# DavidHan008/SLAM-1

Measured on AMD Instinct MI355X. Metric: frames/sec tracking+local-BA @1280x720, higher is better.
Workload: dtype u8+f32+f64

## Files before the change

slam-1_amd/csrc/ba.hip:

```cpp
#include "common.hpp"

#include <cmath>

namespace {

typedef double d4 __attribute__((ext_vector_type(4)));

__device__ __forceinline__ void st_sc1(double* p, double v) {
  __hip_atomic_store(p, v, __ATOMIC_RELAXED, __HIP_MEMORY_SCOPE_AGENT);
}
__device__ __forceinline__ double ld_sc1(const double* p) {
  return __hip_atomic_load(const_cast<double*>(p), __ATOMIC_RELAXED, __HIP_MEMORY_SCOPE_AGENT);
}
__device__ __forceinline__ unsigned ticket_add(uint32_t* p) {
  return __hip_atomic_fetch_add(p, 1u, __ATOMIC_RELAXED, __HIP_MEMORY_SCOPE_AGENT);
}
__device__ __forceinline__ void ticket_reset(uint32_t* p) {
  __hip_atomic_store(p, 0u, __ATOMIC_RELAXED, __HIP_MEMORY_SCOPE_AGENT);
}

constexpr double kClamp = 5000.0;
constexpr double kDiagMin = 1e-6, kDiagMax = 1e32;
constexpr double kLamMin = 1e-16, kLamMax = 1e32;
constexpr int kBS = 256;
// ... 37 lines not shown
  const double omc = 1.0 - c;
  double R[3][3];
  R[0][0] = c + omc * v0 * v0; R[0][1] = -s * v2 + omc * v0 * v1; R[0][2] = s * v1 + omc * v0 * v2;
  R[1][0] = s * v2 + omc * v1 * v0; R[1][1] = c + omc * v1 * v1; R[1][2] = -s * v0 + omc * v1 * v2;
  R[2][0] = -s * v1 + omc * v2 * v0; R[2][1] = s * v0 + omc * v2 * v1; R[2][2] = c + omc * v2 * v2;
  const double th2 = w0 * w0 + w1 * w1 + w2 * w2;
  const double W[3][3] = {{0.0, -w2, w1}, {w2, 0.0, -w0}, {-w1, w0, 0.0}};
  const double w[3] = {w0, w1, w2};
  double A[3][3];
  for (int i = 0; i < 3; ++i)
    for (int k = 0; k < 3; ++k) {
      double acc = w[i] * w[k];
      for (int j = 0; j < 3; ++j) acc += R[j][i] * W[j][k];
      A[i][k] = acc - W[i][k];
    }
  o[0] = c; o[1] = s; o[2] = omc;
  o[3] = v0; o[4] = v1; o[5] = v2;
  for (int i = 0; i < 9; ++i) o[6 + i] = R[i / 3][i % 3];
  for (int i = 0; i < 9; ++i) o[15 + i] = A[i / 3][i % 3];
  o[24] = th2 < 1e-24 ? 0.0 : -1.0 / th2;
  o[25] = th2 < 1e-24 ? 1.0 : 0.0;
  for (int i = 0; i < 6; ++i) o[26 + i] = cam[3 + i];
}

template <bool JAC>
__device__ __forceinline__ void reproject_pre(const double* __restrict__ cr,
                                              const double* __restrict__ X,
                                              const double* __restrict__ q, double r[2],
                                              double J[2][12]) {
  const double c = cr[0], s = cr[1], omc = cr[2];
  const double v0 = cr[3], v1 = cr[4], v2 = cr[5];
  const double X0 = X[0], X1 = X[1], X2 = X[2];
  const double dot = X0 * v0 + X1 * v1 + X2 * v2;
  const double cx0 = v1 * X2 - v2 * X1;
  const double cx1 = v2 * X0 - v0 * X2;
  const double cx2 = v0 * X1 - v1 * X0;
  const double dk = dot * omc;
  const double RX0 = c * X0 + s * cx0 + dk * v0;
  const double RX1 = c * X1 + s * cx1 + dk * v1;
  const double RX2 = c * X2 + s * cx2 + dk * v2;
  const double P0 = RX0 + cr[26], P1 = RX1 + cr[27], P2 = RX2 + cr[28];
  const double p0 = -P0 / P2, p1 = -P1 / P2;
  const double f = cr[29], k1 = cr[30], k2 = cr[31];
  const double n = p0 * p0 + p1 * p1;
  const double rad = 1.0 + k1 * n + k2 * (n * n);
  const double sc = rad * f;
  r[0] = p0 * sc - q[0];
  r[1] = p1 * sc - q[1];
  if constexpr (JAC) {
    double R[3][3], A[3][3];
    for (int i = 0; i < 9; ++i) {
      R[i / 3][i % 3] = cr[6 + i];
      A[i / 3][i % 3] = cr[15 + i];
    }
    double dR[3][3];
    if (cr[25] != 0.0) {
      dR[0][0] = 0.0;  dR[0][1] = RX2;  dR[0][2] = -RX1;
      dR[1][0] = -RX2; dR[1][1] = 0.0;  dR[1][2] = RX0;
      dR[2][0] = RX1;  dR[2][1] = -RX0; dR[2][2] = 0.0;
    } else {
      const double Xs[3][3] = {{0.0, -X2, X1}, {X2, 0.0, -X0}, {-X1, X0, 0.0}};
      double B[3][3];
      for (int i = 0; i < 3; ++i)
        for (int k = 0; k < 3; ++k)
          B[i][k] = Xs[i][0] * A[0][k] + Xs[i][1] * A[1][k] + Xs[i][2] * A[2][k];
      const double inv = cr[24];
      for (int i = 0; i < 3; ++i)
        for (int k = 0; k < 3; ++k)
          dR[i][k] = (R[i][0] * B[0][k] + R[i][1] * B[1][k] + R[i][2] * B[2][k]) * inv;
    }
    const double iz = 1.0 / P2;
    const double dpP[2][3] = {{-iz, 0.0, P0 * iz * iz}, {0.0, -iz, P1 * iz * iz}};
    const double g2 = 2.0 * f * (k1 + 2.0 * k2 * n);
    const double Dp[2][2] = {{sc + g2 * p0 * p0, g2 * p0 * p1}, {g2 * p1 * p0, sc + g2 * p1 * p1}};
    double D[2][3];
    for (int a = 0; a < 2; ++a)
      for (int k = 0; k < 3; ++k) D[a][k] = Dp[a][0] * dpP[0][k] + Dp[a][1] * dpP[1][k];
    const double pp[2] = {p0, p1};
    for (int a = 0; a < 2; ++a) {
      for (int k = 0; k < 3; ++k) {
        J[a][k] = D[a][0] * dR[0][k] + D[a][1] * dR[1][k] + D[a][2] * dR[2][k];
        J[a][3 + k] = D[a][k];
        J[a][9 + k] = D[a][0] * R[0][k] + D[a][1] * R[1][k] + D[a][2] * R[2][k];
      }
      J[a][6] = pp[a] * rad;
      J[a][7] = pp[a] * (f * n);
      J[a][8] = pp[a] * (f * n * n);
    }
  }
}

template <bool JAC>
__device__ __forceinline__ void reproject(const double* __restrict__ cam,
                                          const double* __restrict__ X,
                                          const double* __restrict__ q, double r[2],
                                          double J[2][12]) {
  double cr[kCamRec];
  cam_prep(cam, cr);
  reproject_pre<JAC>(cr, X, q, r, J);
}

template <bool JAC>
__device__ __forceinline__ void clamp_rows(double r[2], double J[2][12]) {
#pragma unroll
  for (int comp = 0; comp < 2; ++comp) {
    const double rc = r[comp];
    if (fabs(rc) > kClamp) {
      const double arc = fabs(rc);
      const double half = comp == 0 ? 613.0 : 185.0;
      if constexpr (JAC) {
        const double a = (half * 2.0) / arc;
        double Jc[12];
        for (int k = 0; k < 12; ++k) Jc[k] = J[comp][k];
        for (int row = 0; row < 2; ++row) {
          const double ratio = r[row] / rc;
          for (int k = 0; k < 12; ++k) J[row][k] = a * (J[row][k] - ratio * Jc[k]);
        }
      }
      r[0] = r[0] / arc * half * 2.0;
      r[1] = r[1] / arc * half * 2.0;
    }
  }
}

__device__ __forceinline__ void hold_cols(double J[2][12], unsigned fx) {
#pragma unroll
  for (int i = 0; i < 9; ++i)
    if ((fx >> i) & 1u) J[0][i] = J[1][i] = 0.0;
}
template <int H>
__device__ __forceinline__ void hold_cols_half(double Jh[2][6], unsigned fx) {
#pragma unroll
  for (int i = 0; i < (H == 0 ? 6 : 3); ++i)
    if ((fx >> (6 * H + i)) & 1u) Jh[0][i] = Jh[1][i] = 0.0;
}

template <int H>
__device__ __forceinline__ void reproject_half(const double* __restrict__ cr,
                                               const double* __restrict__ X,
                                               const double* __restrict__ q, double r[2],
                                               double Jh[2][6]) {
  const double c = cr[0], s = cr[1], omc = cr[2];
  const double v0 = cr[3], v1 = cr[4], v2 = cr[5];
  const double X0 = X[0], X1 = X[1], X2 = X[2];
  const double dot = X0 * v0 + X1 * v1 + X2 * v2;
  const double cx0 = v1 * X2 - v2 * X1;
  const double cx1 = v2 * X0 - v0 * X2;
  const double cx2 = v0 * X1 - v1 * X0;
  const double dk = dot * omc;
  const double RX0 = c * X0 + s * cx0 + dk * v0;
  const double RX1 = c * X1 + s * cx1 + dk * v1;
  const double RX2 = c * X2 + s * cx2 + dk * v2;
  const double P0 = RX0 + cr[26], P1 = RX1 + cr[27], P2 = RX2 + cr[28];
  const double p0 = -P0 / P2, p1 = -P1 / P2;
  const double f = cr[29], k1 = cr[30], k2 = cr[31];
  const double n = p0 * p0 + p1 * p1;
  const double rad = 1.0 + k1 * n + k2 * (n * n);
  const double sc = rad * f;
  r[0] = p0 * sc - q[0];
  r[1] = p1 * sc - q[1];
  const double iz = 1.0 / P2;
  const double dpP[2][3] = {{-iz, 0.0, P0 * iz * iz}, {0.0, -iz, P1 * iz * iz}};
  const double g2 = 2.0 * f * (k1 + 2.0 * k2 * n);
  const double Dp[2][2] = {{sc + g2 * p0 * p0, g2 * p0 * p1}, {g2 * p1 * p0, sc + g2 * p1 * p1}};
  double D[2][3];
  for (int a = 0; a < 2; ++a)
    for (int k = 0; k < 3; ++k) D[a][k] = Dp[a][0] * dpP[0][k] + Dp[a][1] * dpP[1][k];
  if constexpr (H == 0) {
    double dR[3][3];
    if (cr[25] != 0.0) {
      dR[0][0] = 0.0;  dR[0][1] = RX2;  dR[0][2] = -RX1;
      dR[1][0] = -RX2; dR[1][1] = 0.0;  dR[1][2] = RX0;
      dR[2][0] = RX1;  dR[2][1] = -RX0; dR[2][2] = 0.0;
    } else {
      double R[3][3], A[3][3];
      for (int i = 0; i < 9; ++i) {
        R[i / 3][i % 3] = cr[6 + i];
        A[i / 3][i % 3] = cr[15 + i];
      }
      const double Xs[3][3] = {{0.0, -X2, X1}, {X2, 0.0, -X0}, {-X1, X0, 0.0}};
      double B[3][3];
      for (int i = 0; i < 3; ++i)
        for (int k = 0; k < 3; ++k)
          B[i][k] = Xs[i][0] * A[0][k] + Xs[i][1] * A[1][k] + Xs[i][2] * A[2][k];
      const double inv = cr[24];
      for (int i = 0; i < 3; ++i)
        for (int k = 0; k < 3; ++k)
          dR[i][k] = (R[i][0] * B[0][k] + R[i][1] * B[1][k] + R[i][2] * B[2][k]) * inv;
    }
    for (int a = 0; a < 2; ++a)
      for (int k = 0; k < 3; ++k) {
        Jh[a][k] = D[a][0] * dR[0][k] + D[a][1] * dR[1][k] + D[a][2] * dR[2][k];
        Jh[a][3 + k] = D[a][k];
      }
  } else {
    double R[3][3];
    for (int i = 0; i < 9; ++i) R[i / 3][i % 3] = cr[6 + i];
    const double pp[2] = {p0, p1};
    for (int a = 0; a < 2; ++a) {
      Jh[a][0] = pp[a] * rad;
      Jh[a][1] = pp[a] * (f * n);
      Jh[a][2] = pp[a] * (f * n * n);
      for (int k = 0; k < 3; ++k) Jh[a][3 + k] = D[a][0] * R[0][k] + D[a][1] * R[1][k] + D[a][2] * R[2][k];
    }
  }
#pragma unroll
  for (int comp = 0; comp < 2; ++comp) {
    const double rc = r[comp];
    if (fabs(rc) > kClamp) {
      const double arc = fabs(rc);
      const double half = comp == 0 ? 613.0 : 185.0;
      const double a = (half * 2.0) / arc;
      double Jc[6];
      for (int k = 0; k < 6; ++k) Jc[k] = Jh[comp][k];
      for (int row = 0; row < 2; ++row) {
        const double ratio = r[row] / rc;
        for (int k = 0; k < 6; ++k) Jh[row][k] = a * (Jh[row][k] - ratio * Jc[k]);
      }
      r[0] = r[0] / arc * half * 2.0;
      r[1] = r[1] / arc * half * 2.0;
    }
  }
}

__device__ __forceinline__ double block_sum(double v, double* lds) {
  for (int off = 32; off > 0; off >>= 1) v += __shfl_down(v, off, 64);
  const int lane = threadIdx.x & 63, wid = threadIdx.x >> 6;
  if (lane == 0) lds[wid] = v;
  __syncthreads();
  double s = 0.0;
  if (threadIdx.x == 0) {
    const int nw = (blockDim.x + 63) >> 6;
    for (int w = 0; w < nw; ++w) s += lds[w];
  }
  __syncthreads();
  return s;
}

__global__ __launch_bounds__(kBS) void k_residual(const double* __restrict__ cams,
                                                  const double* __restrict__ pts,
                                                  const int32_t* __restrict__ ci,
                                                  const int32_t* __restrict__ pi,
                                                  const double* __restrict__ qs, int n_obs,
                                                  double* __restrict__ resid,
                                                  double* __restrict__ jac) {
  const int o = blockIdx.x * kBS + threadIdx.x;
  if (o >= n_obs) return;
  double r[2], J[2][12];
  if (jac) {
    reproject<true>(cams + 9 * ci[o], pts + 3 * pi[o], qs + 2 * o, r, J);
    clamp_rows<true>(r, J);
    for (int a = 0; a < 2; ++a)
      for (int k = 0; k < 12; ++k) jac[(size_t)o * 24 + a * 12 + k] = J[a][k];
  } else {
    reproject<false>(cams + 9 * ci[o], pts + 3 * pi[o], qs + 2 * o, r, J);
    clamp_rows<false>(r, J);
  }
  resid[2 * o] = r[0];
  resid[2 * o + 1] = r[1];
}

__device__ __forceinline__ int cur_of(const double* state) {
  return state[SLAM_BA_ST_CUR] != 0.0 ? 1 : 0;
}

__device__ __forceinline__ double clampd(double d) { return fmin(fmax(d, kDiagMin), kDiagMax); }

constexpr int kDenseMaxN = 120;
__host__ __device__ __forceinline__ bool sys_packed(int n_cams) { return 9 * n_cams > kDenseMaxN; }
__host__ __device__ __forceinline__ long long sys_vec_off(int n_cams, int n_blocks) {
  return sys_packed(n_cams) ? 81ll * n_blocks : 81ll * n_cams * n_cams;
}


struct PtSchur {
  double V00 = 0, V01 = 0, V02 = 0, V11 = 0, V12 = 0, V22 = 0, g0 = 0, g1 = 0, g2 = 0;
  double d[3], iv[6], e[3];
  __device__ __forceinline__ void acc(double j0, double j1, double j2, double rr) {
    V00 += j0 * j0; V01 += j0 * j1; V02 += j0 * j2;
    V11 += j1 * j1; V12 += j1 * j2; V22 += j2 * j2;
    g0 -= j0 * rr; g1 -= j1 * rr; g2 -= j2 * rr;
  }
  __device__ __forceinline__ void solve(double lam);
};
__device__ __forceinline__ void PtSchur::solve(double lam) {
  d[0] = clampd(V00); d[1] = clampd(V11); d[2] = clampd(V22);
  const double a00 = V00 + lam * d[0], a11 = V11 + lam * d[1], a22 = V22 + lam * d[2];
  const double a01 = V01, a02 = V02, a12 = V12;
  const double c00 = a11 * a22 - a12 * a12;
  const double c01 = a02 * a12 - a01 * a22;
  const double c02 = a01 * a12 - a02 * a11;
  const double c11 = a00 * a22 - a02 * a02;
  const double c12 = a01 * a02 - a00 * a12;
  const double c22 = a00 * a11 - a01 * a01;
  const double det = a00 * c00 + a01 * c01 + a02 * c02;
  const double id = det != 0.0 ? 1.0 / det : 0.0;
  iv[0] = c00 * id; iv[1] = c01 * id; iv[2] = c02 * id;
  iv[3] = c11 * id; iv[4] = c12 * id; iv[5] = c22 * id;
  e[0] = iv[0] * g0 + iv[1] * g1 + iv[2] * g2;
  e[1] = iv[1] * g0 + iv[3] * g1 + iv[4] * g2;
  e[2] = iv[2] * g0 + iv[4] * g1 + iv[5] * g2;
}

constexpr int kCPart = 112;
constexpr int kGrp = 128;
constexpr int kLinWG = 256;
constexpr int kSlotLds = 128;
constexpr int kPairLds = 1024;

struct LinLds {
  double jc[kGrp][18];
  double w[kGrp][27];
  double ru[kGrp][4];
  double pt[kGrp][9];
  int lpt[kGrp];
  int cobs[kGrp];
  int cptr[kSlotLds];
  int bptr[kSlotLds];
  int pairs[kPairLds];
  unsigned fx[kGrp];
};

__device__ __forceinline__ void y_row(const double* W, const double* Vi, int i, double y[3]) {
  const double a = W[3 * i], b = W[3 * i + 1], c = W[3 * i + 2];
  y[0] = a * Vi[0] + b * Vi[1] + c * Vi[2];
  y[1] = a * Vi[1] + b * Vi[3] + c * Vi[4];
  y[2] = a * Vi[2] + b * Vi[4] + c * Vi[5];
}

__device__ __forceinline__ void lin_slots(const slam_ba_problem& p, LinLds& L, int cs0, int ncs,
                                          int bs0, int nbs, const int* cptr, int coff,
                                          const int* bptr, int boff, const int* pairs) {
  const int t = threadIdx.x;
  const int* cobs = L.cobs;
  for (int item = t; item < 9 * (ncs + nbs); item += kLinWG) {
    const int sl = item / 9, i = item - 9 * sl;
    double acc[9];
#pragma unroll
    for (int j = 0; j < 9; ++j) acc[j] = 0.0;
    if (sl < ncs) {
      const int s = cs0 + sl;
      double vr = 0.0, vu = 0.0, vd = 0.0, cost = 0.0;
      const int qb = cptr[sl] - coff, qe = cptr[sl + 1] - coff;
      int k = cobs[qb < qe ? qb : 0], lk = L.lpt[k];
      for (int q = qb; q < qe; ++q) {
        const int kn = cobs[q + 1 < qe ? q + 1 : q], lkn = L.lpt[kn];
        const double* jc = L.jc[k];
        const double* W = L.w[k];
        double y[3];
        y_row(W, L.pt[lk] + 3, i, y);
        const double a0 = jc[i], a1 = jc[9 + i];
#pragma unroll
        for (int j = 0; j < 9; ++j) {
          const double u = __builtin_fma(a0, jc[j], a1 * jc[9 + j]);
          const double v = __builtin_fma(y[0], W[3 * j], __builtin_fma(y[1], W[3 * j + 1], y[2] * W[3 * j + 2]));
          acc[j] += u - v;
        }
        const double r0 = L.ru[k][0], r1 = L.ru[k][1];
        vr = __builtin_fma(a0, r0, __builtin_fma(a1, r1, vr));
        vu = __builtin_fma(a0, L.ru[k][2], __builtin_fma(a1, L.ru[k][3], vu));
        vd = __builtin_fma(a0, a0, __builtin_fma(a1, a1, vd));
        cost = __builtin_fma(r0, r0, __builtin_fma(r1, r1, cost));
        k = kn;
        lk = lkn;
      }
      double* out = p.cpart + (size_t)p.cslot_row[s] * kCPart;
#pragma unroll
      for (int j = 0; j < 9; ++j) out[9 * i + j] = acc[j];
      out[81 + i] = vr;
      out[90 + i] = vu;
      out[99 + i] = vd;
      if (i == 0) out[108] = cost;
    } else {
      const int sb = sl - ncs, s = bs0 + sb;
      const int qb = bptr[sb] - boff, qe = bptr[sb + 1] - boff;
      int pr = pairs[qb < qe ? qb : 0], lk = L.lpt[pr & 0xffff];
      for (int q = qb; q < qe; ++q) {
        const int prn = pairs[q + 1 < qe ? q + 1 : q], lkn = L.lpt[prn & 0xffff];
        const int k1 = pr & 0xffff, k2 = pr >> 16;
        double y[3];
        y_row(L.w[k1], L.pt[lk] + 3, i, y);
        const double* W2 = L.w[k2];
#pragma unroll
        for (int j = 0; j < 9; ++j)
          acc[j] = __builtin_fma(y[0], W2[3 * j], __builtin_fma(y[1], W2[3 * j + 1], __builtin_fma(y[2], W2[3 * j + 2], acc[j])));
        pr = prn;
        lk = lkn;
      }
      double* out = p.bpart + (size_t)p.bslot_row[s] * 81;
#pragma unroll
      for (int j = 0; j < 9; ++j) out[9 * i + j] = acc[j];
    }
  }
}

#ifdef SLAM_LIN_PROFILE
#define LIN_T(i) const uint64_t lin_t##i = __builtin_amdgcn_s_memtime()
#else
#define LIN_T(i) (void)0
#endif
__global__ __launch_bounds__(kLinWG) void k_linearize(BaBatch bat) {
  BA_PROB_X(bat);
  const int g = bx;
  if (g >= p.n_grps) return;
  lm_wave_priority();
  __shared__ LinLds L;
  LIN_T(0);
  const int p0 = p.grp_ptr[g], p1 = p.grp_ptr[g + 1];
  const int o0 = p.pt_ptr[p0], o1 = p.pt_ptr[p1];
  const int t = threadIdx.x;
  const int o = o0 + t;
  const bool has = t < kGrp && o < o1;
  const int cur = cur_of(p.state);
  const int cs0 = p.grp_cslot[g], ncs = p.grp_cslot[g + 1] - cs0;
  const int bs0 = p.grp_bslot[g], nbs = p.grp_bslot[g + 1] - bs0;
  const int cb0 = p.cslot_obs_ptr[cs0], pb0 = p.bslot_pair_ptr[bs0];
  const int npairs = p.bslot_pair_ptr[bs0 + nbs] - pb0;
  const bool fit_c = ncs < kSlotLds, fit_b = nbs < kSlotLds, fit_p = npairs <= kPairLds;
  if (fit_c && t <= ncs) L.cptr[t] = p.cslot_obs_ptr[cs0 + t] - cb0;
  if (fit_b && t <= nbs) L.bptr[t] = p.bslot_pair_ptr[bs0 + t] - pb0;
  if (t < kGrp && t < o1 - o0) L.cobs[t] = p.cslot_obs[cb0 + t];
  if (fit_p)
    for (int q = t; q < npairs; q += kLinWG) L.pairs[q] = p.bslot_pairs[pb0 + q];
  double r[2], J[2][12];
  if (has) {
    const int pt = p.obs_pt[o];
    reproject_pre<true>(p.camrec[cur] + kCamRec * p.obs_cam[o], p.pts[cur] + 3 * pt,
                        p.obs_q + 2 * o, r, J);
    clamp_rows<true>(r, J);
#pragma unroll
    for (int a = 0; a < 2; ++a) {
#pragma unroll
      for (int i = 0; i < 9; ++i) L.jc[t][9 * a + i] = J[a][i];
#pragma unroll
      for (int c = 0; c < 3; ++c) L.w[t][3 * a + c] = J[a][9 + c];
      L.w[t][6 + a] = r[a];
      L.ru[t][a] = r[a];
    }
    L.lpt[t] = pt - p0;
  }
  __syncthreads();
  if (p.cam_fixed != nullptr) {
    for (int sl = t; sl < ncs; sl += kLinWG) {
      const unsigned fx = p.cam_fixed[p.cslot_cam[cs0 + sl]];
      const int qe = p.cslot_obs_ptr[cs0 + sl + 1] - cb0;
      for (int q = p.cslot_obs_ptr[cs0 + sl] - cb0; q < qe; ++q) L.fx[L.cobs[q]] = fx;
    }
    __syncthreads();
    if (has) {
      const unsigned fx = L.fx[t];
      if (fx) {
        hold_cols(J, fx);
#pragma unroll
        for (int i = 0; i < 9; ++i)
          if ((fx >> i) & 1u) L.jc[t][i] = L.jc[t][9 + i] = 0.0;
      }
    }
  }
  LIN_T(1);
  const double lam = p.state[SLAM_BA_ST_LAMBDA];
  if (t < p1 - p0) {
    const int pt = p0 + t;
    PtSchur ps;
    for (int k = p.pt_ptr[pt] - o0; k < p.pt_ptr[pt + 1] - o0; ++k) {
#pragma unroll
      for (int a = 0; a < 2; ++a) ps.acc(L.w[k][3 * a], L.w[k][3 * a + 1], L.w[k][3 * a + 2], L.w[k][6 + a]);
    }
    ps.solve(lam);
#pragma unroll
    for (int k = 0; k < 3; ++k) L.pt[t][k] = ps.e[k];
#pragma unroll
    for (int k = 0; k < 6; ++k) L.pt[t][3 + k] = ps.iv[k];
  }
  __syncthreads();
  if (has) {
    const double* e = L.pt[L.lpt[t]];
#pragma unroll
    for (int i = 0; i < 9; ++i)
#pragma unroll
      for (int c = 0; c < 3; ++c) L.w[t][3 * i + c] = J[0][i] * J[0][9 + c] + J[1][i] * J[1][9 + c];
    L.ru[t][2] = J[0][9] * e[0] + J[0][10] * e[1] + J[0][11] * e[2];
    L.ru[t][3] = J[1][9] * e[0] + J[1][10] * e[1] + J[1][11] * e[2];
  }
  __syncthreads();
  LIN_T(2);
  if (fit_c && fit_b && fit_p)
    lin_slots(p, L, cs0, ncs, bs0, nbs, L.cptr, 0, L.bptr, 0, L.pairs);
  else
    lin_slots(p, L, cs0, ncs, bs0, nbs, p.cslot_obs_ptr + cs0, cb0, p.bslot_pair_ptr + bs0, pb0,
              p.bslot_pairs + pb0);
#ifdef SLAM_LIN_PROFILE
  __builtin_amdgcn_s_waitcnt(0);
  __syncthreads();
  LIN_T(3);
  if (g == 7 && t == 0) {
    p.state[12] = (double)(lin_t1 - lin_t0);
    p.state[13] = (double)(lin_t2 - lin_t1);
    p.state[14] = (double)(lin_t3 - lin_t2);
    p.state[15] = (double)(ncs * 100 + nbs);
  }
#endif
}

constexpr int kMObs = 120, kMPts = 16, kMCams = 7, kMRows = 64;
constexpr int kMWG = 256;
constexpr int kSgMeta = 24;
constexpr int kMObsS = kMObs + 1;
struct alignas(16) MLds {
  double jc[18][kMObsS];
  double jp[6][kMObsS];
  double ru[4][kMObsS];
  double vi[kMPts][6];
  double e[kMPts][3];
  double yt[kMPts][3][kMRows];
  double wt[kMPts][3][kMRows];
  double cam[kMCams][kCamRec];
  double X[kMPts][3];
  double zero;
  int optr[kMPts + 1];
  int lpt[kMObs];
  int la[kMObs];
  int cobs[kMObs];
  int cptr[8];
  unsigned fx[kMCams];
  int crow[kMCams];
  int bab[kMCams * (kMCams - 1) / 2], brow[kMCams * (kMCams - 1) / 2];
};
static_assert(sizeof(MLds) <= 80 * 1024, "k_lin_mfma: two workgroups per CU");
static_assert(9 * kMCams <= kMRows, "k_lin_mfma: 9m rows in 4 tile rows");
static_assert(kMCams * kCamRec + kMCams <= kMWG, "k_lin_mfma: a lane per record entry and per mask word");
static_assert(2 * kMPts * 3 * kMRows >= kMRows * kMRows + kMCams * 256, "staging aliases yt/wt");

#ifdef SLAM_LINM_PROFILE
__device__ unsigned long long g_linm_stamp[4096][8];
#define LINM_DECL() unsigned long long linm_prev = __builtin_amdgcn_s_memtime(), linm_acc[7] = {0, 0, 0, 0, 0, 0, 0}
#define LINM_T(i)                                                  \
  do {                                                             \
    if (threadIdx.x == 0) {                                        \
      const unsigned long long linm_now = __builtin_amdgcn_s_memtime(); \
      linm_acc[i] += linm_now - linm_prev;                         \
      linm_prev = linm_now;                                        \
    }                                                              \
  } while (0)
#define LINM_END()                                                               \
  do {                                                                           \
    if (threadIdx.x == 0 && blockIdx.x + 1024 * blockIdx.y < 4096)               \
      for (int linm_i = 0; linm_i < 7; ++linm_i)                                 \
        g_linm_stamp[blockIdx.x + 1024 * blockIdx.y][linm_i] = linm_acc[linm_i]; \
  } while (0)
#else
#define LINM_DECL() (void)0
#define LINM_T(i) (void)0
#define LINM_END() (void)0
#endif

struct AsmTab {
  const int32_t* need;
  int32_t* cnt;
  const int32_t* cam_dblk;
  const int32_t* row_blk;
  int n_empty;
  const int32_t* empty;
  __device__ explicit AsmTab(const slam_ba_problem& p) {
    const int nb = p.n_blocks;
    need = p.asm_tab;
    cnt = p.asm_tab + nb;
    cam_dblk = p.asm_tab + 2 * nb;
    row_blk = cam_dblk + p.n_cams;
    n_empty = row_blk[p.n_bslots];
    empty = row_blk + p.n_bslots + 1;
  }
};

__device__ void fold_rows_sum(const double* __restrict__ part, int stride, int rb, int re, int n,
                              double* red, double* out) {
  const int t = threadIdx.x;
  const int nparts = kMWG / n, k = t / n, e = t - k * n;
  if (k < nparts) {
    double a[4] = {0.0, 0.0, 0.0, 0.0};
    int r = rb + k;
    for (; r + 3 * nparts < re; r += 4 * nparts) {
      double v[4];
#pragma unroll
      for (int u = 0; u < 4; ++u) v[u] = ld_sc1(part + (size_t)(r + u * nparts) * stride + e);
#pragma unroll
      for (int u = 0; u < 4; ++u) a[u] += v[u];
    }
    for (int u = 0; r < re; r += nparts, ++u) a[u] += ld_sc1(part + (size_t)r * stride + e);
    red[k * n + e] = (a[0] + a[1]) + (a[2] + a[3]);
  }
  __syncthreads();
  if (t < n) {
    double v = 0.0;
    for (int q = 0; q < nparts; ++q) v += red[q * n + t];
    out[t] = v;
  }
  __syncthreads();
}

__device__ void fold_block(const slam_ba_problem& p, int blk, double* scratch) {
  double* red = scratch;
  double* sh = scratch + 3 * kCPart;
  double* sb = sh + kCPart;
  const int c1 = p.blocks[2 * blk], c2 = p.blocks[2 * blk + 1];
  const int C9 = 9 * p.n_cams, t = threadIdx.x;
  double* S = p.sys;
  double* bvec = S + sys_vec_off(p.n_cams, p.n_blocks);
  double* gvec = bvec + C9;
  double* diagU = gvec + C9;
  double* costc = diagU + C9;
  const bool diag = c1 == c2;
  const int bb = p.blk_bslot_ptr[blk], be = p.blk_bslot_ptr[blk + 1];
  if (diag) fold_rows_sum(p.cpart, kCPart, p.cam_cslot_ptr[c1], p.cam_cslot_ptr[c1 + 1], 109, red, sh);
  if (be > bb) {
    fold_rows_sum(p.bpart, 81, bb, be, 81, red, sb);
  } else if (t < 81) {
    sb[t] = 0.0;
  }
  __syncthreads();
  if (sys_packed(p.n_cams)) {
    if (t < 81) S[(size_t)blk * 81 + t] = diag ? sh[t] - (sb[t] + sb[9 * (t % 9) + t / 9]) : -sb[t];
  } else if (t < 81) {
    const int i = t / 9, j = t - 9 * (t / 9);
    if (diag) {
      S[(size_t)(9 * c1 + i) * C9 + 9 * c1 + j] = sh[t] - (sb[t] + sb[9 * j + i]);
    } else {
      S[(size_t)(9 * c1 + i) * C9 + 9 * c2 + j] = -sb[t];
      S[(size_t)(9 * c2 + j) * C9 + 9 * c1 + i] = -sb[t];
    }
  }
  if (diag && t < 9) {
    gvec[9 * c1 + t] = -sh[81 + t];
    bvec[9 * c1 + t] = -sh[81 + t] - sh[90 + t];
    diagU[9 * c1 + t] = sh[99 + t];
  }
  if (diag && t == 0) costc[c1] = sh[108];
  __syncthreads();
}

__device__ void fold_zero_block(const slam_ba_problem& p, int blk, int t0, int nt) {
  const int c1 = p.blocks[2 * blk], c2 = p.blocks[2 * blk + 1];
  const int C9 = 9 * p.n_cams;
  double* S = p.sys;
  double* bvec = S + sys_vec_off(p.n_cams, p.n_blocks);
  for (int e = t0; e < 81; e += nt) {
    const int i = e / 9, j = e - 9 * (e / 9);
    if (sys_packed(p.n_cams)) {
      S[(size_t)blk * 81 + e] = 0.0;
    } else {
      S[(size_t)(9 * c1 + i) * C9 + 9 * c2 + j] = 0.0;
      S[(size_t)(9 * c2 + j) * C9 + 9 * c1 + i] = 0.0;
    }
  }
  if (c1 == c2)
    for (int e = t0; e < 28; e += nt) {
      if (e < 27) bvec[(size_t)(e / 9) * C9 + 9 * c1 + e % 9] = 0.0;
      else bvec[3 * (size_t)C9 + c1] = 0.0;
    }
}

__device__ void lin_fold_assemble(const slam_ba_problem& p, const int* cams, int m, int nb,
                                  const int* brow, double* scratch) {
  const AsmTab A(p);
  __shared__ int done[kMCams + kMCams * (kMCams - 1) / 2];
  __shared__ int ndone;
  __builtin_amdgcn_s_waitcnt(0);
  __syncthreads();
  if (threadIdx.x == 0) {
    int n = 0;
    for (int q = 0; q < m + nb; ++q) {
      const int blk = q < m ? A.cam_dblk[cams[q]] : A.row_blk[brow[q - m]];
      const int old = (int)ticket_add(reinterpret_cast<uint32_t*>(A.cnt + blk));
      if (old == A.need[blk] - 1) {
        done[n++] = blk;
        __hip_atomic_store(A.cnt + blk, 0, __ATOMIC_RELAXED, __HIP_MEMORY_SCOPE_AGENT);
      }
    }
    ndone = n;
  }
  __syncthreads();
  for (int q = 0; q < ndone; ++q) fold_block(p, done[q], scratch);
}

__global__ __launch_bounds__(kMWG) void k_lin_mfma(BaBatch bat) {
  BA_PROB_X(bat);
  const int sg = bx;
  if (sg >= p.n_sgrps) return;
  LINM_DECL();
  lm_wave_priority();
  __shared__ MLds L;
  if (p.asm_tab != nullptr) {
    const AsmTab A(p);
    for (int q = sg; q < A.n_empty; q += p.n_sgrps) fold_zero_block(p, A.empty[q], threadIdx.x, kMWG);
  }
  const int t = threadIdx.x, lane = t & 63;
  const int wid = __builtin_amdgcn_readfirstlane(t >> 6);
  const int* sm = p.sg_meta + kSgMeta * sg;
  const int ch0 = sm[0], ch1 = sm[1], cs0 = sm[2], m = sm[3], bs0 = sm[4], nb = sm[5];
  const int nt = (9 * m + 15) >> 4;
  const int cur = cur_of(p.state);
  const double lam = p.state[SLAM_BA_ST_LAMBDA];
  const bool held = p.cam_fixed != nullptr;
  if (t < kMCams * kCamRec) {
    const int a = t / kCamRec, k = t - kCamRec * (t / kCamRec);
    const int c = a < m ? sm[10 + a] : -1;
    if (c >= 0) L.cam[a][k] = p.camrec[cur][(size_t)kCamRec * c + k];
  } else if (held && t - kMCams * kCamRec < m) {
    const int a = t - kMCams * kCamRec;
    L.fx[a] = p.cam_fixed[sm[10 + a]];
  }
  if (t == 0) L.zero = 0.0;
  if (t < m) L.crow[t] = p.cslot_row[cs0 + t];
  if (t >= 64 && t - 64 < nb) {
    L.bab[t - 64] = p.bslot_ab[bs0 + t - 64];
    L.brow[t - 64] = p.bslot_row[bs0 + t - 64];
  }
  int tI[3], tJ[3];
  int ntl = 0;
  {
    int s = 0;
    for (int I = 0; I < nt; ++I)
      for (int J = I; J < nt; ++J, ++s)
        if ((s & 3) == wid && ntl < 3) {
          tI[ntl] = I;
          tJ[ntl] = J;
          ++ntl;
        }
  }
  const int nza = (m > wid) + (m > wid + 4);
  int tRow[3], tCol[3];
#pragma unroll
  for (int s = 0; s < 3; ++s) {
    tRow[s] = 16 * (s < ntl ? tI[s] : 0) + (lane & 15);
    tCol[s] = 16 * (s < ntl ? tJ[s] : 0) + (lane & 15);
  }
  d4 acc[3], zacc[2];
#pragma unroll
  for (int s = 0; s < 3; ++s) acc[s] = d4{0.0, 0.0, 0.0, 0.0};
#pragma unroll
  for (int s = 0; s < 2; ++s) zacc[s] = d4{0.0, 0.0, 0.0, 0.0};
  const int mi = lane & 15, mk = lane >> 4;

  struct ChunkIn {
    double q0, q1, xv;
    int meta, pp, cp;
  };
  auto load_in = [&](int ch, int p0, int p1, int o0, int o1) {
    ChunkIn in{0.0, 0.0, 0.0, 0, 0, 0};
    const int nobs = o1 - o0, npts = p1 - p0;
    const int ko = t & 127;
    if (ko < nobs) {
      in.q0 = p.obs_q[2 * (o0 + ko)];
      in.q1 = p.obs_q[2 * (o0 + ko) + 1];
    }
    if (t < nobs) in.meta = p.obs_meta[o0 + t];
    if (t < 3 * npts) in.xv = p.pts[cur][3 * p0 + t];
    if (t >= 128 && t - 128 <= npts) in.pp = p.pt_ptr[p0 + t - 128] - o0;
    if (t < 8) in.cp = p.chk_cptr[8 * ch + t];
    return in;
  };
  int p0 = sm[6], p1 = sm[7], o0 = sm[8], o1 = sm[9];
  int np0 = 0, np1 = 0, no0 = 0, no1 = 0;
  if (ch0 + 1 < ch1) {
    np0 = p.grp_ptr[ch0 + 1];
    np1 = p.grp_ptr[ch0 + 2];
    no0 = p.chk_optr[ch0 + 1];
    no1 = p.chk_optr[ch0 + 2];
  }
  ChunkIn in = load_in(ch0, p0, p1, o0, o1);
  for (int ch = ch0; ch < ch1; ++ch) {
    const int nobs = o1 - o0, npts = p1 - p0;
    const double q0 = in.q0, q1 = in.q1;
    __syncthreads();
    if (t < nobs) {
      L.lpt[t] = in.meta & 255;
      L.la[t] = (in.meta >> 8) & 255;
      L.cobs[t] = in.meta >> 16;
    }
    if (t < 3 * npts) (&L.X[0][0])[t] = in.xv;
    if (t >= 128 && t - 128 <= npts) L.optr[t - 128] = in.pp;
    if (t < 8) L.cptr[t] = in.cp;
    {
      typedef double dbl2 __attribute__((ext_vector_type(2)));
      dbl2* y2 = reinterpret_cast<dbl2*>(&L.yt[0][0][0]);
      dbl2* w2 = reinterpret_cast<dbl2*>(&L.wt[0][0][0]);
      const int n2 = npts * 3 * kMRows / 2;
      for (int i = t; i < n2; i += kMWG) {
        y2[i] = dbl2{0.0, 0.0};
        w2[i] = dbl2{0.0, 0.0};
      }
    }
    __syncthreads();
    int nnp0 = 0, nnp1 = 0, nno0 = 0, nno1 = 0;
    if (ch + 1 < ch1) {
      in = load_in(ch + 1, np0, np1, no0, no1);
      if (ch + 2 < ch1) {
        nnp0 = p.grp_ptr[ch + 2];
        nnp1 = p.grp_ptr[ch + 3];
        nno0 = p.chk_optr[ch + 2];
        nno1 = p.chk_optr[ch + 3];
      }
    }
    LINM_T(1);
    {
      const int k = t & 127;
      if (k < nobs) {
        const double q[2] = {q0, q1};
        double r[2], Jh[2][6];
        if (t < 128) {
          reproject_half<0>(L.cam[L.la[k]], L.X[L.lpt[k]], q, r, Jh);
          if (held) hold_cols_half<0>(Jh, L.fx[L.la[k]]);
#pragma unroll
          for (int a = 0; a < 2; ++a) {
#pragma unroll
            for (int i = 0; i < 6; ++i) L.jc[9 * a + i][k] = Jh[a][i];
            L.ru[a][k] = r[a];
          }
        } else {
          reproject_half<1>(L.cam[L.la[k]], L.X[L.lpt[k]], q, r, Jh);
          if (held) hold_cols_half<1>(Jh, L.fx[L.la[k]]);
#pragma unroll
          for (int a = 0; a < 2; ++a) {
#pragma unroll
            for (int i = 0; i < 3; ++i) L.jc[9 * a + 6 + i][k] = Jh[a][i];
#pragma unroll
            for (int c = 0; c < 3; ++c) L.jp[3 * a + c][k] = Jh[a][3 + c];
          }
        }
      }
    }
    __syncthreads();
    LINM_T(2);
    if (t < npts) {
      PtSchur ps;
      for (int k = L.optr[t]; k < L.optr[t + 1]; ++k) {
#pragma unroll
        for (int a = 0; a < 2; ++a) ps.acc(L.jp[3 * a][k], L.jp[3 * a + 1][k], L.jp[3 * a + 2][k], L.ru[a][k]);
      }
      ps.solve(lam);
#pragma unroll
      for (int k = 0; k < 3; ++k) L.e[t][k] = ps.e[k];
#pragma unroll
      for (int k = 0; k < 6; ++k) L.vi[t][k] = ps.iv[k];
    }
    __syncthreads();
    LINM_T(3);
    {
      const int h = t >> 7, k0 = t & 127;
      const bool lead = k0 < nobs && (k0 == 0 || L.lpt[k0 - 1] != L.lpt[k0] ||
                                      L.la[k0 - 1] != L.la[k0]);
      if (lead) {
        const int lp = L.lpt[k0], a = L.la[k0];
        const int ib = h ? 5 : 0, ie = h ? 9 : 5;
        double W[5][3];
#pragma unroll
        for (int i = 0; i < 5; ++i)
#pragma unroll
          for (int c = 0; c < 3; ++c) W[i][c] = 0.0;
        for (int k = k0; k < nobs && L.lpt[k] == lp && L.la[k] == a; ++k) {
#pragma unroll
          for (int i = 0; i < 5; ++i) {
            if (ib + i >= ie) break;
#pragma unroll
            for (int c = 0; c < 3; ++c)
              W[i][c] += L.jc[ib + i][k] * L.jp[c][k] + L.jc[9 + ib + i][k] * L.jp[3 + c][k];
          }
        }
        const double* vi = L.vi[lp];
        const double V[3][3] = {{vi[0], vi[1], vi[2]}, {vi[1], vi[3], vi[4]}, {vi[2], vi[4], vi[5]}};
#pragma unroll
        for (int i = 0; i < 5; ++i) {
          if (ib + i >= ie) break;
          const int row = 9 * a + ib + i;
#pragma unroll
          for (int c = 0; c < 3; ++c) {
            const int pos = (row + 16 * ((3 * lp + c) & 3)) & (kMRows - 1);
            L.wt[lp][c][pos] = W[i][c];
            L.yt[lp][c][pos] = W[i][0] * V[0][c] + W[i][1] * V[1][c] + W[i][2] * V[2][c];
          }
        }
      }
      if (h == 0 && k0 < nobs) {
        const double* e = L.e[L.lpt[k0]];
        L.ru[2][k0] = L.jp[0][k0] * e[0] + L.jp[1][k0] * e[1] + L.jp[2][k0] * e[2];
        L.ru[3][k0] = L.jp[3][k0] * e[0] + L.jp[4][k0] * e[1] + L.jp[5][k0] * e[2];
      }
    }
    __syncthreads();
    LINM_T(4);
    {
      const double* Yf = &L.yt[0][0][0];
      const double* Wf = &L.wt[0][0][0];
      const int nk = 3 * npts;
      for (int k0 = 0; k0 < nk; k0 += 16) {
        double av[4][3], bv[4][3];
#pragma unroll
        for (int u = 0; u < 4; ++u) {
          const int kk = min(k0 + 4 * u + mk, 3 * kMPts - 1);
#pragma unroll
          for (int s = 0; s < 3; ++s) {
            av[u][s] = Yf[kk * kMRows + ((tRow[s] + 16 * mk) & (kMRows - 1))];
            bv[u][s] = Wf[kk * kMRows + ((tCol[s] + 16 * mk) & (kMRows - 1))];
          }
        }
#pragma unroll
        for (int u = 0; u < 4; ++u) {
          const bool on = k0 + 4 * u + mk < nk;
#pragma unroll
          for (int s = 0; s < 3; ++s) {
            const bool o = on && s < ntl;
            acc[s] = __builtin_amdgcn_mfma_f64_16x16x4f64(o ? av[u][s] : 0.0, o ? bv[u][s] : 0.0,
                                                         acc[s], 0, 0, 0);
          }
        }
      }
    }
    {
      const int row = mk & 1;
      int qb[2], qe[2];
#pragma unroll
      for (int s = 0; s < 2; ++s) {
        const int a = wid + 4 * s;
        qb[s] = s < nza ? L.cptr[a] : 0;
        qe[s] = s < nza ? L.cptr[a + 1] : 0;
      }
      const int nsteps = max(qe[0] - qb[0], qe[1] - qb[1]);
      for (int q = 0; q < nsteps; q += 8) {
        double z[2][4];
        bool ok[2][4];
#pragma unroll
        for (int s = 0; s < 2; ++s)
#pragma unroll
          for (int u = 0; u < 4; ++u) {
            const int qq = qb[s] + q + 2 * u + (mk >> 1);
            ok[s][u] = qq < qe[s];
            const int k = L.cobs[ok[s][u] ? qq : 0];
            const double* src = mi < 9 ? &L.jc[9 * row + mi][k]
                                : mi < 11 ? &L.ru[row + 2 * (mi - 9)][k] : &L.zero;
            z[s][u] = *src;
          }
#pragma unroll
        for (int u = 0; u < 4; ++u)
#pragma unroll
          for (int s = 0; s < 2; ++s) {
            const double zv = ok[s][u] ? z[s][u] : 0.0;
            zacc[s] = __builtin_amdgcn_mfma_f64_16x16x4f64(zv, zv, zacc[s], 0, 0, 0);
          }
      }
    }
    p0 = np0; p1 = np1; o0 = no0; o1 = no1;
    np0 = nnp0; np1 = nnp1; no0 = nno0; no1 = nno1;
    LINM_T(5);
  }
  __syncthreads();
  double* T = &L.yt[0][0][0];
  double* Z = T + kMRows * kMRows;
#pragma unroll
  for (int s = 0; s < 3; ++s) {
    if (s >= ntl) break;
#pragma unroll
    for (int r = 0; r < 4; ++r)
      T[(16 * tI[s] + mk + 4 * r) * kMRows + 16 * tJ[s] + mi] = acc[s][r];
  }
#pragma unroll
  for (int s = 0; s < 2; ++s) {
    if (s >= nza) break;
#pragma unroll
    for (int r = 0; r < 4; ++r) Z[(wid + 4 * s) * 256 + (mk + 4 * r) * 16 + mi] = zacc[s][r];
  }
  __syncthreads();
  const bool fold = p.asm_tab != nullptr;
  for (int q = t; q < m * 109; q += kMWG) {
    const int a = q / 109, e = q - 109 * (q / 109);
    const double* Za = Z + a * 256;
    double v;
    if (e < 81) {
      const int i = e / 9, j = e - 9 * (e / 9);
      const int row = 9 * a + i, col = 9 * a + j;
      const double tv = (row >> 4) <= (col >> 4) ? T[row * kMRows + col] : T[col * kMRows + row];
      v = Za[i * 16 + j] - tv;
    } else if (e < 90) {
      v = Za[(e - 81) * 16 + 9];
    } else if (e < 99) {
      v = Za[(e - 90) * 16 + 10];
    } else if (e < 108) {
      v = Za[(e - 99) * 17];
    } else {
      v = Za[9 * 16 + 9];
    }
    double* cp = p.cpart + (size_t)L.crow[a] * kCPart + e;
    if (fold) st_sc1(cp, v);
    else *cp = v;
  }
  for (int q = t; q < 81 * nb; q += kMWG) {
    const int pr = q / 81, e = q - 81 * (q / 81);
    const int ab = L.bab[pr], a = ab & 255, b = ab >> 8;
    const int i = e / 9, j = e - 9 * (e / 9);
    const double v = T[(9 * a + i) * kMRows + 9 * b + j];
    double* bp = p.bpart + (size_t)L.brow[pr] * 81 + e;
    if (fold) st_sc1(bp, v);
    else *bp = v;
  }
  LINM_T(6);
  if (p.asm_tab != nullptr) lin_fold_assemble(p, sm + 10, m, nb, L.brow, &L.jc[0][0]);
  LINM_END();
}

#ifndef SLAM_ASM_WG
#define SLAM_ASM_WG 1024
#endif
constexpr int kAsmWG = SLAM_ASM_WG;
static_assert(kAsmWG >= 128 && kAsmWG % 64 == 0, "SLAM_ASM_WG");
__device__ void rows_sum(const double* __restrict__ part, int stride, int rb, int re, int n,
                         double (*red)[kCPart], double* out) {
  const int t = threadIdx.x;
  const int nparts = kAsmWG / n, k = t / n, e = t - k * n;
  if (k < nparts) {
    double a[8] = {0, 0, 0, 0, 0, 0, 0, 0};
    int r = rb + k;
    for (; r + 7 * nparts < re; r += 8 * nparts) {
      double v[8];
#pragma unroll
      for (int u = 0; u < 8; ++u) v[u] = part[(size_t)(r + u * nparts) * stride + e];
#pragma unroll
      for (int u = 0; u < 8; ++u) a[u] += v[u];
    }
    for (int u = 0; r < re; r += nparts, ++u) a[u] += part[(size_t)r * stride + e];
    red[k][e] = ((a[0] + a[1]) + (a[2] + a[3])) + ((a[4] + a[5]) + (a[6] + a[7]));
  }
  __syncthreads();
  if (t < n) {
    double v = 0.0;
    for (int q = 0; q < nparts; ++q) v += red[q][t];
    out[t] = v;
  }
  __syncthreads();
}

__global__ __launch_bounds__(kAsmWG) void k_assemble(BaBatch bat) {
  BA_PROB_X(bat);
  if (bx >= (p.asm_act != nullptr ? p.n_asm_act : p.n_blocks)) return;
  lm_wave_priority();
  __shared__ double red[kAsmWG / 81][kCPart];
  __shared__ double sh[kCPart];
  __shared__ double sb[81];
  const int blk = p.asm_act != nullptr ? p.asm_act[bx] : bx;
  if (p.asm_act != nullptr) {
    const int32_t* listed = p.asm_act + p.n_asm_act;
    const int32_t* camrows = listed + p.n_blocks;
    const size_t ns = (size_t)p.n_blocks * 81, c9 = 9 * (size_t)p.n_cams, nv = ns + 3 * c9 + p.n_cams;
    for (size_t i = (size_t)bx * kAsmWG + threadIdx.x; i < nv; i += (size_t)p.n_asm_act * kAsmWG) {
      if (i < ns) {
        if (!listed[i / 81]) p.sys[i] = -0.0;
      } else {
        const size_t j = i - ns;
        const int cam = j < 3 * c9 ? (int)((j % c9) / 9) : (int)(j - 3 * c9);
        if (!camrows[cam]) p.sys[i] = j < 2 * c9 ? -0.0 : 0.0;
      }
    }
  }
  const int c1 = p.blocks[2 * blk], c2 = p.blocks[2 * blk + 1];
  const int C9 = 9 * p.n_cams;
  double* S = p.sys;
  double* bvec = S + sys_vec_off(p.n_cams, p.n_blocks);
  double* gvec = bvec + C9;
  double* diagU = gvec + C9;
  double* costc = diagU + C9;
  const int t = threadIdx.x;
  const bool diag = c1 == c2;
  const int bb = p.blk_bslot_ptr[blk], be = p.blk_bslot_ptr[blk + 1];
  if (!diag && be == bb) {
    if (t < 81) {
      if (sys_packed(p.n_cams)) {
        S[(size_t)blk * 81 + t] = -0.0;
      } else {
        const int i = t / 9, j = t - 9 * (t / 9);
        S[(size_t)(9 * c1 + i) * C9 + 9 * c2 + j] = -0.0;
        S[(size_t)(9 * c2 + j) * C9 + 9 * c1 + i] = -0.0;
      }
    }
    return;
  }
  if (diag) rows_sum(p.cpart, kCPart, p.cam_cslot_ptr[c1], p.cam_cslot_ptr[c1 + 1], 109, red, sh);
  if (!diag || be > bb) {
    rows_sum(p.bpart, 81, bb, be, 81, red, sb);
  } else if (t < 81) {
    sb[t] = 0.0;
  }
  __syncthreads();
  if (sys_packed(p.n_cams)) {
    if (t < 81) S[(size_t)blk * 81 + t] = diag ? sh[t] - (sb[t] + sb[9 * (t % 9) + t / 9]) : -sb[t];
  } else if (t < 81) {
    const int i = t / 9, j = t - 9 * (t / 9);
    if (diag) {
      S[(size_t)(9 * c1 + i) * C9 + 9 * c1 + j] = sh[t] - (sb[t] + sb[9 * j + i]);
    } else {
      S[(size_t)(9 * c1 + i) * C9 + 9 * c2 + j] = -sb[t];
      S[(size_t)(9 * c2 + j) * C9 + 9 * c1 + i] = -sb[t];
    }
  }
  if (diag && t < 9) {
    gvec[9 * c1 + t] = -sh[81 + t];
    bvec[9 * c1 + t] = -sh[81 + t] - sh[90 + t];
    diagU[9 * c1 + t] = sh[99 + t];
  }
  if (diag && t == 0) costc[c1] = sh[108];
}

constexpr int kLdsMaxN = kDenseMaxN;
constexpr int kSolveHdr = 32;

struct EpiSrc {
  const double *g, *dU, *cam, *costc;
};
#ifdef SLAM_FLOW_PROFILE
__device__ unsigned long long g_flow_epi[4];
#endif

__device__ __forceinline__ void block_sum2(double& a, double& b, double* lds) {
  for (int off = 32; off > 0; off >>= 1) {
    a += __shfl_down(a, off, 64);
    b += __shfl_down(b, off, 64);
  }
  const int lane = threadIdx.x & 63, wid = threadIdx.x >> 6;
  if (lane == 0) {
    lds[wid] = a;
    lds[16 + wid] = b;
  }
  __syncthreads();
  if (threadIdx.x == 0) {
    const int nw = (blockDim.x + 63) >> 6;
    a = 0.0;
    b = 0.0;
    for (int w = 0; w < nw; ++w) {
      a += lds[w];
      b += lds[16 + w];
    }
  }
  __syncthreads();
}

template <bool GLOBAL = false>
__device__ void solve_epilogue(const slam_ba_problem& p, const double* x, bool ok, double* red,
                               const EpiSrc& e, int fail_code = 1) {
  const int C9 = 9 * p.n_cams, t = threadIdx.x;
  double* state = p.state;
  const double lam = state[SLAM_BA_ST_LAMBDA];
  const int cur = cur_of(state);
  double pc = 0.0, cost = 0.0;
  if constexpr (GLOBAL) {
    const int nt = blockDim.x;
    for (int i0 = t; i0 < C9; i0 += 8 * nt) {
      double xv[8], cv[8], uv[8], gv[8];
#pragma unroll
      for (int q = 0; q < 8; ++q) {
        const int i = min(i0 + q * nt, C9 - 1);
        xv[q] = x[i];
        cv[q] = e.cam[i];
        uv[q] = e.dU[i];
        gv[q] = e.g[i];
      }
#pragma unroll
      for (int q = 0; q < 8; ++q) {
        const int i = i0 + q * nt;
        if (i < C9) {
          const double d = ok ? xv[q] : 0.0;
          p.delta_c[i] = d;
          p.cams[1 - cur][i] = cv[q] + d;
          pc += d * (lam * clampd(uv[q]) * d + gv[q]);
        }
      }
    }
    for (int c = t; c < p.n_cams; c += nt) cost += e.costc[c];
    block_sum2(pc, cost, red);
#ifdef SLAM_FLOW_PROFILE
    if (t == 0) g_flow_epi[2] = wall_clock64();
#endif
  } else {
    for (int i = t; i < C9; i += blockDim.x) {
      const double d = ok ? x[i] : 0.0;
      p.delta_c[i] = d;
      p.cams[1 - cur][i] = e.cam[i] + d;
      pc += d * (lam * clampd(e.dU[i]) * d + e.g[i]);
    }
// ... 2490 lines not shown
```

Baseline: 22390.

## Parallelize per-point Schur accumulation across 16 lanes with DPP row gathers

```diff
diff --git a/slam-1_amd/csrc/ba.hip b/slam-1_amd/csrc/ba.hip
--- a/slam-1_amd/csrc/ba.hip
+++ b/slam-1_amd/csrc/ba.hip
@@ -363,6 +363,34 @@
   e[2] = iv[2] * g0 + iv[4] * g1 + iv[5] * g2;
 }
 
+__device__ __forceinline__ double pt_comp(const double* jr, int stride, int kb, int ke, int j) {
+  const int ia = j < 3 ? 0 : j < 5 ? 1 : j < 6 ? 2 : j - 6;
+  const int ib = j < 3 ? j : j < 5 ? j - 2 : 2;
+  const bool isg = j >= 6;
+  const double* xr[2] = {jr + ia * stride, jr + (3 + ia) * stride};
+  const double* yr[2] = {jr + (isg ? 6 : ib) * stride, jr + (isg ? 7 : 3 + ib) * stride};
+  double v = 0.0;
+  for (int k = kb; k < ke; k += 4) {
+    double x[4][2], y[4][2];
+#pragma unroll
+    for (int u = 0; u < 4; ++u) {
+      const int kk = min(k + u, ke - 1);
+#pragma unroll
+      for (int a = 0; a < 2; ++a) {
+        x[u][a] = xr[a][kk];
+        y[u][a] = yr[a][kk];
+      }
+    }
+#pragma unroll
+    for (int u = 0; u < 4; ++u) {
+      if (k + u >= ke) break;
+#pragma unroll
+      for (int a = 0; a < 2; ++a) v += (isg ? -x[u][a] : x[u][a]) * y[u][a];
+    }
+  }
+  return v;
+}
+
 constexpr int kCPart = 112;
 constexpr int kGrp = 128;
 constexpr int kLinWG = 256;
@@ -566,6 +594,7 @@
 constexpr int kMObs = 120, kMPts = 16, kMCams = 7, kMRows = 64;
 constexpr int kMWG = 256;
 constexpr int kSgMeta = 24;
+constexpr int kNoObs = 255;
 constexpr int kMObsS = kMObs + 1;
 struct alignas(16) MLds {
   double jc[18][kMObsS];
@@ -583,11 +612,16 @@
   int la[kMObs];
   int cobs[kMObs];
   int cptr[8];
+  uint8_t kfirst[kMPts][8];
   unsigned fx[kMCams];
   int crow[kMCams];
   int bab[kMCams * (kMCams - 1) / 2], brow[kMCams * (kMCams - 1) / 2];
 };
 static_assert(sizeof(MLds) <= 80 * 1024, "k_lin_mfma: two workgroups per CU");
+static_assert(offsetof(MLds, ru) == offsetof(MLds, jp) + 6 * kMObsS * sizeof(double),
+              "k_lin_mfma: (B) reads Jp and r as the rows of one array");
+static_assert(kMObs <= kNoObs && kMCams <= 8 && kMPts * 8 <= kMWG, "k_lin_mfma: kfirst");
+static_assert(16 * kMPts <= kMWG && 2 * kMCams <= 16, "k_lin_mfma: 16 lanes per point in (B), (C)");
 static_assert(9 * kMCams <= kMRows, "k_lin_mfma: 9m rows in 4 tile rows");
 static_assert(kMCams * kCamRec + kMCams <= kMWG, "k_lin_mfma: a lane per record entry and per mask word");
 static_assert(2 * kMPts * 3 * kMRows >= kMRows * kMRows + kMCams * 256, "staging aliases yt/wt");
@@ -829,6 +863,15 @@
     no1 = p.chk_optr[ch0 + 2];
   }
   ChunkIn in = load_in(ch0, p0, p1, o0, o1);
+  {
+    typedef double dbl2 __attribute__((ext_vector_type(2)));
+    dbl2* y2 = reinterpret_cast<dbl2*>(&L.yt[0][0][0]);
+    dbl2* w2 = reinterpret_cast<dbl2*>(&L.wt[0][0][0]);
+    for (int i = t; i < kMPts * 3 * kMRows / 2; i += kMWG) {
+      y2[i] = dbl2{0.0, 0.0};
+      w2[i] = dbl2{0.0, 0.0};
+    }
+  }
   for (int ch = ch0; ch < ch1; ++ch) {
     const int nobs = o1 - o0, npts = p1 - p0;
     const double q0 = in.q0, q1 = in.q1;
@@ -841,17 +884,12 @@
     if (t < 3 * npts) (&L.X[0][0])[t] = in.xv;
     if (t >= 128 && t - 128 <= npts) L.optr[t - 128] = in.pp;
     if (t < 8) L.cptr[t] = in.cp;
-    {
-      typedef double dbl2 __attribute__((ext_vector_type(2)));
-      dbl2* y2 = reinterpret_cast<dbl2*>(&L.yt[0][0][0]);
-      dbl2* w2 = reinterpret_cast<dbl2*>(&L.wt[0][0][0]);
-      const int n2 = npts * 3 * kMRows / 2;
-      for (int i = t; i < n2; i += kMWG) {
-        y2[i] = dbl2{0.0, 0.0};
-        w2[i] = dbl2{0.0, 0.0};
-      }
-    }
+    int tl = t;
+    asm volatile("" : "+v"(tl));
+    if (tl < kMPts * 8) (&L.kfirst[0][0])[tl] = kNoObs;
     __syncthreads();
+    if (tl < nobs && (tl == 0 || L.lpt[tl - 1] != L.lpt[tl] || L.la[tl - 1] != L.la[tl]))
+      L.kfirst[L.lpt[tl]][L.la[tl]] = (uint8_t)tl;
     int nnp0 = 0, nnp1 = 0, nno0 = 0, nno1 = 0;
     if (ch + 1 < ch1) {
       in = load_in(ch + 1, np0, np1, no0, no1);
@@ -892,33 +930,53 @@
     }
     __syncthreads();
     LINM_T(2);
-    if (t < npts) {
+    {
+      tl = t;
+      asm volatile("" : "+v"(tl));
+      const int lp = tl >> 4, j = tl & 15;
+      double v = 0.0;
+      if (lp < npts && j < 9) v = pt_comp(&L.jp[0][0], kMObsS, L.optr[lp], L.optr[lp + 1], j);
       PtSchur ps;
-      for (int k = L.optr[t]; k < L.optr[t + 1]; ++k) {
-#pragma unroll
-        for (int a = 0; a < 2; ++a) ps.acc(L.jp[3 * a][k], L.jp[3 * a + 1][k], L.jp[3 * a + 2][k], L.ru[a][k]);
-      }
-      ps.solve(lam);
-#pragma unroll
-      for (int k = 0; k < 3; ++k) L.e[t][k] = ps.e[k];
-#pragma unroll
-      for (int k = 0; k < 6; ++k) L.vi[t][k] = ps.iv[k];
+      auto row_lane = [](double x, auto sh) {
+        constexpr int kSh = decltype(sh)::value;
+        union { double d; int w[2]; } a, b;
+        a.d = x;
+        b.w[0] = __builtin_amdgcn_update_dpp(0, a.w[0], 0x100 + kSh, 0xF, 0xF, false);
+        b.w[1] = __builtin_amdgcn_update_dpp(0, a.w[1], 0x100 + kSh, 0xF, 0xF, false);
+        return b.d;
+      };
+      ps.V00 = v;
+      ps.V01 = row_lane(v, std::integral_constant<int, 1>{});
+      ps.V02 = row_lane(v, std::integral_constant<int, 2>{});
+      ps.V11 = row_lane(v, std::integral_constant<int, 3>{});
+      ps.V12 = row_lane(v, std::integral_constant<int, 4>{});
+      ps.V22 = row_lane(v, std::integral_constant<int, 5>{});
+      ps.g0 = row_lane(v, std::integral_constant<int, 6>{});
+      ps.g1 = row_lane(v, std::integral_constant<int, 7>{});
+      ps.g2 = row_lane(v, std::integral_constant<int, 8>{});
+      if (lp < npts && j == 0) {
+        ps.solve(lam);
+#pragma unroll
+        for (int k = 0; k < 3; ++k) L.e[lp][k] = ps.e[k];
+#pragma unroll
+        for (int k = 0; k < 6; ++k) L.vi[lp][k] = ps.iv[k];
+      }
     }
     __syncthreads();
     LINM_T(3);
     {
-      const int h = t >> 7, k0 = t & 127;
-      const bool lead = k0 < nobs && (k0 == 0 || L.lpt[k0 - 1] != L.lpt[k0] ||
-                                      L.la[k0 - 1] != L.la[k0]);
-      if (lead) {
-        const int lp = L.lpt[k0], a = L.la[k0];
-        const int ib = h ? 5 : 0, ie = h ? 9 : 5;
+      const int lp = tl >> 4, a = (tl & 15) >> 1, hh = tl & 1;
+      if (lp < npts && a < m) {
+        const int ke = L.optr[lp + 1];
+        const int kf = L.kfirst[lp][a];
+        const int ib = hh ? 5 : 0, ie = hh ? 9 : 5;
+        const bool seen = kf != kNoObs;
         double W[5][3];
 #pragma unroll
         for (int i = 0; i < 5; ++i)
 #pragma unroll
           for (int c = 0; c < 3; ++c) W[i][c] = 0.0;
-        for (int k = k0; k < nobs && L.lpt[k] == lp && L.la[k] == a; ++k) {
+        for (int k = kf; k < ke && L.la[k] == a; ++k) {
 #pragma unroll
           for (int i = 0; i < 5; ++i) {
             if (ib + i >= ie) break;
@@ -936,11 +994,13 @@
 #pragma unroll
           for (int c = 0; c < 3; ++c) {
             const int pos = (row + 16 * ((3 * lp + c) & 3)) & (kMRows - 1);
+            const double y = W[i][0] * V[0][c] + W[i][1] * V[1][c] + W[i][2] * V[2][c];
             L.wt[lp][c][pos] = W[i][c];
-            L.yt[lp][c][pos] = W[i][0] * V[0][c] + W[i][1] * V[1][c] + W[i][2] * V[2][c];
+            L.yt[lp][c][pos] = seen ? y : 0.0;
           }
         }
       }
+      const int h = t >> 7, k0 = t & 127;
       if (h == 0 && k0 < nobs) {
         const double* e = L.e[L.lpt[k0]];
         L.ru[2][k0] = L.jp[0][k0] * e[0] + L.jp[1][k0] * e[1] + L.jp[2][k0] * e[2];
```

Result: faster. 22700 (median of 6 runs) (+1.4%).
